# kjedrzejewski/video-cycle_gan-upscaling

Hardware: AMD Instinct MI355X
Metric: upscaled frames/s (train step, G+D fwd+bwd) at 256->512 (higher is better)
Workload: dtype f32; 1 GPU; C2: make_upscaler_orig((512,512,3),k=3,x2,res=9) + PatchGAN-70, batch 8/GPU, gan2 wiring, Wasserstein + pixel-MSE, faithful 3-call step incl. predict pass; global_batch=8, frame=256x256->512x512, parallelism=dp1, launch=hipGraph replay

## Files before the change

video-cycle_gan-upscaling_amd/csrc/conv_transpose.hip:

```cpp
#include "vcg_common.hpp"
#include <type_traits>

namespace {

struct ConvTParams {
    const float* x;
    const float* w;
    float* y;
    const float* bias;
    const float* prelu;
    const float* residual;
    int n, cin, h, w_, cout, oh, ow;
    int tiles_x, tiles_y, co_blocks;
    int act;
    float alpha;
};

constexpr int phase_of(int k, int cb) { return (((k - cb) % 2) + 2) % 2; }
constexpr int d_of(int k, int cb) { return (k - cb - phase_of(k, cb)) / 2; }
constexpr int dmin_of(int K, int cb) { int m = 1000; for (int k = 0; k < K; ++k) m = d_of(k, cb) < m ? d_of(k, cb) : m; return m; }
constexpr int dmax_of(int K, int cb) { int m = -1000; for (int k = 0; k < K; ++k) m = d_of(k, cb) > m ? d_of(k, cb) : m; return m; }

template <int K, int CBY, int CBX, int CK, int MT>
struct ConvTCfg {
    static constexpr int QROWS = 4;
    static constexpr int DMINY = dmin_of(K, CBY), DMAXY = dmax_of(K, CBY);
    static constexpr int DMINX = dmin_of(K, CBX), DMAXX = dmax_of(K, CBX);
    static constexpr int NDY = DMAXY - DMINY + 1, NDX = DMAXX - DMINX + 1;
    static constexpr int NR = QROWS + DMAXY - DMINY;
    static constexpr int NC = 32 + DMAXX - DMINX;
    static constexpr int PLANE = NR * NC;
    static constexpr int T = K * K;
    static constexpr int IN_ELEMS = CK * PLANE;
    static constexpr int MB = 32 * MT;
    static constexpr int W_ELEMS = CK * T * MB;
    static constexpr int IN_PT = (IN_ELEMS + 255) / 256;
    static constexpr int W_PT = (W_ELEMS + 255) / 256;
    static constexpr size_t LDS_BYTES = (size_t)(IN_ELEMS + W_ELEMS) * sizeof(float);
};

template <int K, int CBY, int CBX, int CK, int MT>
__global__ __launch_bounds__(256, (MT == 1 ? 2 : 1)) void convt_kernel(const ConvTParams p) {
    using C = ConvTCfg<K, CBY, CBX, CK, MT>;
    extern __shared__ __attribute__((aligned(16))) float smem[];
    float* s_in = smem;
    float* s_w = smem + C::IN_ELEMS;

    const int tid = threadIdx.x, lane = tid & 63, wv = tid >> 6;
    const int half = lane >> 5, l31 = lane & 31;
    int b = blockIdx.x;
    const int cb = b % p.co_blocks; b /= p.co_blocks;
    const int tx = b % p.tiles_x;   b /= p.tiles_x;
    const int ty = b % p.tiles_y;   b /= p.tiles_y;
    const int n = b;
    const int qx0 = tx * 32, qy0 = ty * C::QROWS, co0 = cb * C::MB;
    const int gy0 = qy0 - C::DMAXY, gx0 = qx0 - C::DMAXX;
    const float* xn = p.x + (size_t)n * p.cin * p.h * p.w_;

    float rin[C::IN_PT], rw[C::W_PT];
    unsigned in_off[C::IN_PT];
#pragma unroll
    for (int i = 0; i < C::IN_PT; ++i) {
        const int e = tid + i * 256;
        unsigned off = VCG_OOB;
        if (e < C::IN_ELEMS) {
            const int ci = e / C::PLANE, rem = e % C::PLANE;
            const int r = rem / C::NC, c = rem % C::NC;
            const int gy = gy0 + r, gx = gx0 + c;
            if (gy >= 0 && gy < p.h && gx >= 0 && gx < p.w_) off = 4u * (unsigned)((ci * p.h + gy) * p.w_ + gx);
        }
        in_off[i] = off;
    }
    const int hw = p.h * p.w_;
    unsigned w_off[C::W_PT];
#pragma unroll
    for (int i = 0; i < C::W_PT; ++i) {
        const int e = tid + i * 256;
        const int m = e % C::MB, q = e / C::MB;
        const int t = q % C::T, ci = q / C::T;
        const int col = co0 + m < p.cout ? co0 + m : p.cout - 1;
        w_off[i] = e < C::W_ELEMS ? 4u * (unsigned)((t * p.cin + ci) * p.cout + col) : VCG_OOB;
    }
    const size_t wbytes = (size_t)C::T * p.cin * p.cout * sizeof(float);
    auto load_chunk = [&](int ci0) {
        const vcg_rsrc rx = make_rsrc(xn + (size_t)ci0 * hw, (size_t)(p.cin - ci0) * hw * sizeof(float));
#pragma unroll
        for (int i = 0; i < C::IN_PT; ++i) rin[i] = buf_load(rx, in_off[i]);
        const vcg_rsrc rwt = make_rsrc(p.w + (size_t)ci0 * p.cout, wbytes - (size_t)ci0 * p.cout * sizeof(float));
#pragma unroll
        for (int i = 0; i < C::W_PT; ++i) rw[i] = buf_load(rwt, w_off[i]);
    };
    auto store_chunk = [&]() {
#pragma unroll
        for (int i = 0; i < C::IN_PT; ++i) {
            const int e = tid + i * 256;
            if (e < C::IN_ELEMS) s_in[e] = rin[i];
        }
#pragma unroll
        for (int i = 0; i < C::W_PT; ++i) {
            const int e = tid + i * 256;
            if (e < C::W_ELEMS) s_w[e] = rw[i];
        }
    };

    f32x16 acc[2][2][MT];
#pragma unroll
    for (int a = 0; a < 2; ++a)
#pragma unroll
        for (int c = 0; c < 2; ++c)
#pragma unroll
            for (int m = 0; m < MT; ++m)
#pragma unroll
                for (int r = 0; r < 16; ++r) acc[a][c][m][r] = 0.f;

    const float* bbase = s_in + half * C::PLANE + wv * C::NC + l31;
    const float* abase = s_w + half * C::T * C::MB + l31;

    const int nchunks = (p.cin + CK - 1) / CK;
    load_chunk(0);
    for (int c = 0; c < nchunks; ++c) {
        __syncthreads();
        store_chunk();
        __syncthreads();
        if (c + 1 < nchunks) load_chunk((c + 1) * CK);
#pragma unroll
        for (int cp = 0; cp < CK / 2; ++cp) {
            float bv[C::NDY][C::NDX];
#pragma unroll
            for (int iy = 0; iy < C::NDY; ++iy)
#pragma unroll
                for (int ix = 0; ix < C::NDX; ++ix)
                    bv[iy][ix] = bbase[cp * 2 * C::PLANE + (C::DMAXY - (C::DMINY + iy)) * C::NC +
                                       (C::DMAXX - (C::DMINX + ix))];
            float av[C::T][MT];
#pragma unroll
            for (int t = 0; t < C::T; ++t)
#pragma unroll
                for (int mt = 0; mt < MT; ++mt) av[t][mt] = abase[(cp * 2 * C::T + t) * C::MB + mt * 32];
#pragma unroll
            for (int ky = 0; ky < K; ++ky) {
#pragma unroll
                for (int kx = 0; kx < K; ++kx) {
                    const int t = ky * K + kx;
                    const int py = phase_of(ky, CBY), px = phase_of(kx, CBX);
                    const int iy = d_of(ky, CBY) - C::DMINY, ix = d_of(kx, CBX) - C::DMINX;
#pragma unroll
                    for (int mt = 0; mt < MT; ++mt) acc[py][px][mt] = mfma32(av[t][mt], bv[iy][ix], acc[py][px][mt]);
                }
            }
        }
    }

    const int qy = qy0 + wv, qx = qx0 + l31;
    const bool vec_ok = (p.ow % 2) == 0;
    const bool full = vec_ok && (co0 + C::MB <= p.cout) && (2 * (qy0 + C::QROWS) <= p.oh) && (2 * (qx0 + 32) <= p.ow);
    const int plane = p.oh * p.ow;
    const size_t img = (size_t)n * p.cout * plane;
    float* yimg = p.y + img;
    const float* rimg = p.residual ? p.residual + img : nullptr;
    const int ob = (co0 + 4 * half) * plane + (2 * qy) * p.ow + 2 * qx;
    const float* bp = p.bias ? p.bias : vcg_zero_word;
    const int bmask = p.bias ? ~0 : 0;
    const bool is_prelu = p.act == VCG_ACT_PRELU;
    const float* ap = is_prelu ? p.prelu : vcg_zero_word;
    const int amask = is_prelu ? ~0 : 0;
    const float slope_u = (p.act == VCG_ACT_LRELU) ? p.alpha : 1.f;
    auto emit = [&](auto guard_tag, auto res_tag) {
        constexpr bool GUARD = decltype(guard_tag)::value, RES = decltype(res_tag)::value;
#pragma unroll
        for (int mt = 0; mt < MT; ++mt) {
#pragma unroll
            for (int r = 0; r < 16; ++r) {
                const int row = mt * 32 + mfma_row(r, lane);
                const int co = co0 + row;
                const bool co_ok = !GUARD || co < p.cout;
                const int cs = co_ok ? co : co0;
                const float bvv = bp[cs & bmask];
                const float pa = ap[cs & amask];
                const float al = is_prelu ? pa : slope_u;
#pragma unroll
                for (int py = 0; py < 2; ++py) {
                    const int o = ob + (row - 4 * half) * plane + py * p.ow;
                    float v0 = acc[py][0][mt][r] + bvv, v1 = acc[py][1][mt][r] + bvv;
                    v0 = v0 >= 0.f ? v0 : v0 * al;
                    v1 = v1 >= 0.f ? v1 : v1 * al;
                    if (!GUARD) {
                        if (RES) { const float2 rr = *reinterpret_cast<const float2*>(rimg + o); v0 += rr.x; v1 += rr.y; }
                        *reinterpret_cast<float2*>(yimg + o) = make_float2(v0, v1);
                    } else {
                        const int oy = 2 * qy + py, ox = 2 * qx;
                        if (co_ok && oy < p.oh && ox < p.ow) {
                            if (vec_ok) {
                                if (RES) { const float2 rr = *reinterpret_cast<const float2*>(rimg + o); v0 += rr.x; v1 += rr.y; }
                                *reinterpret_cast<float2*>(yimg + o) = make_float2(v0, v1);
                            } else {
                                if (RES) v0 += rimg[o];
                                yimg[o] = v0;
                                if (ox + 1 < p.ow) {
                                    if (RES) v1 += rimg[o + 1];
                                    yimg[o + 1] = v1;
                                }
                            }
                        }
                    }
                }
            }
        }
    };
    using T_ = std::true_type;
    using F_ = std::false_type;
    if (full) {
        if (p.residual) emit(F_{}, T_{}); else emit(F_{}, F_{});
    } else {
        if (p.residual) emit(T_{}, T_{}); else emit(T_{}, F_{});
    }
}

template <int K, int CBY, int CBX, int CK, int MT>
int launch_convt(ConvTParams p, hipStream_t st) {
    using C = ConvTCfg<K, CBY, CBX, CK, MT>;
    p.tiles_x = ceil_div(ceil_div(p.ow, 2), 32);
    p.tiles_y = ceil_div(ceil_div(p.oh, 2), C::QROWS);
    p.co_blocks = ceil_div(p.cout, C::MB);
    const long grid = (long)p.tiles_x * p.tiles_y * p.co_blocks * p.n;
    if (grid <= 0 || grid > 0x7fffffffL) return VCG_E_SHAPE;
    auto kern = convt_kernel<K, CBY, CBX, CK, MT>;
    if (int e = vcg_allow_dyn_lds(reinterpret_cast<const void*>(kern), C::LDS_BYTES)) return e;
    hipLaunchKernelGGL(kern, dim3((int)grid), dim3(256), C::LDS_BYTES, st, p);
    VCG_LAUNCH_CHECK();
    return VCG_OK;
}

}

int vcg_internal_convt(const float* x, const float* w, float* y, int n, int cin, int h, int wd, int cout,
                       int oh, int ow, int k, int cby, int cbx, const vcg_epilogue* ep, hipStream_t st) {
    ConvTParams p{};
    p.x = x; p.w = w; p.y = y;
    p.bias = ep ? ep->bias : nullptr;
    p.prelu = ep ? ep->prelu_alpha : nullptr;
    p.residual = ep ? ep->residual : nullptr;
    p.act = ep ? ep->act : VCG_ACT_NONE;
    p.alpha = ep ? ep->act_alpha : 0.f;
    if (p.act == VCG_ACT_PRELU && p.prelu == nullptr) return VCG_E_NULL;
    if (p.act == VCG_ACT_TANH) return VCG_E_UNSUPPORTED;
    p.n = n; p.cin = cin; p.h = h; p.w_ = wd; p.cout = cout; p.oh = oh; p.ow = ow;
    if (n <= 0 || cin <= 0 || cout <= 0 || oh <= 0 || ow <= 0) return VCG_E_SHAPE;
#define VCG_CT(K_, A_, B_, CK_, MT_) if (k == K_ && cby == A_ && cbx == B_) return launch_convt<K_, A_, B_, CK_, MT_>(p, st)
    VCG_CT(3, 0, 0, 16, 1); VCG_CT(3, 0, 1, 16, 1); VCG_CT(3, 1, 0, 16, 1); VCG_CT(3, 1, 1, 16, 1);
    VCG_CT(4, 1, 1, 16, 1);
    VCG_CT(5, 1, 1, 8, 2); VCG_CT(5, 1, 2, 8, 2); VCG_CT(5, 2, 1, 8, 2); VCG_CT(5, 2, 2, 8, 2);
#undef VCG_CT
    return VCG_E_UNSUPPORTED;
}
```

Before: 135.7 frames/s.

## Walk several output-channel blocks per CTA in transposed conv and rework epilogue

Each block now loops over several consecutive output-channel blocks (a walk factor picked from occupancy so the grid still fills the GPU), reusing its input tile position across them. The grid becomes 3D, residual handling becomes a template parameter so the non-residual K=3 kernel can request higher occupancy, and the staging offsets are computed incrementally instead of with divisions. The epilogue uses buffer loads and stores with saturated out-of-bounds offsets, vectorized bias and slope loads, and prefetches the residual. Walking serializes work per block and reloads input chunks per channel block, so it trades parallelism for fewer blocks and less index overhead.

```diff
diff --git a/video-cycle_gan-upscaling_amd/csrc/conv_transpose.hip b/video-cycle_gan-upscaling_amd/csrc/conv_transpose.hip
--- a/video-cycle_gan-upscaling_amd/csrc/conv_transpose.hip
+++ b/video-cycle_gan-upscaling_amd/csrc/conv_transpose.hip
@@ -11,7 +11,8 @@
     const float* prelu;
     const float* residual;
     int n, cin, h, w_, cout, oh, ow;
-    int tiles_x, tiles_y, co_blocks;
+    int tiles_x, co_blocks;
+    int walk;
     int act;
     float alpha;
 };
@@ -39,47 +40,158 @@
     static constexpr size_t LDS_BYTES = (size_t)(IN_ELEMS + W_ELEMS) * sizeof(float);
 };
 
-template <int K, int CBY, int CBX, int CK, int MT>
-__global__ __launch_bounds__(256, (MT == 1 ? 2 : 1)) void convt_kernel(const ConvTParams p) {
+constexpr int CT_OOB = 0x7FFFFFF0;
+__device__ __forceinline__ float2 buf_load2(vcg_rsrc r, int byte_off) {
+    const u32x2 v = __builtin_amdgcn_raw_buffer_load_b64(r, byte_off, 0, 0);
+    return make_float2(__uint_as_float(v.x), __uint_as_float(v.y));
+}
+__device__ __forceinline__ f32x4 buf_load4(vcg_rsrc r, int byte_off) {
+    return __builtin_bit_cast(f32x4, __builtin_amdgcn_raw_buffer_load_b128(r, byte_off, 0, 0));
+}
+__device__ __forceinline__ void buf_store2(vcg_rsrc r, int byte_off, float a, float b) {
+    u32x2 v;
+    v.x = __float_as_uint(a);
+    v.y = __float_as_uint(b);
+    __builtin_amdgcn_raw_buffer_store_b64(v, r, byte_off, 0, 0);
+}
+
+template <int MT, bool RES>
+__device__ __forceinline__ void convt_epilogue(const ConvTParams& p, f32x16 (&acc)[2][2][MT], int n, int co0, int qy, int qx, int half) {
+    constexpr int MB = 32 * MT;
+    const int plane = p.oh * p.ow, plane4 = 4 * plane, ow4 = 4 * p.ow;
+    const int nch = p.cout - co0 < MB ? p.cout - co0 : MB;
+    const size_t blk = ((size_t)n * p.cout + co0) * plane;
+    const size_t blk_bytes = (size_t)nch * plane * sizeof(float);
+    const vcg_rsrc ry = make_rsrc(p.y + blk, blk_bytes);
+    const vcg_rsrc rr = make_rsrc(RES ? p.residual + blk : nullptr, RES ? blk_bytes : 0);
+    const bool is_prelu = p.act == VCG_ACT_PRELU;
+    const vcg_rsrc rbias = make_rsrc(p.bias, p.bias ? (size_t)p.cout * sizeof(float) : 0);
+    const vcg_rsrc rslope = make_rsrc(is_prelu ? p.prelu : nullptr, is_prelu ? (size_t)p.cout * sizeof(float) : 0);
+    const float slope_u = (p.act == VCG_ACT_LRELU) ? p.alpha : 1.f;
+    const int chan4 = 4 * (co0 + 4 * half);
+
+    const int base = (4 * half) * plane4 + (2 * qy) * ow4 + 8 * qx;
+    int vo[2][2];
+#pragma unroll
+    for (int py = 0; py < 2; ++py)
+#pragma unroll
+        for (int px = 0; px < 2; ++px)
+            vo[py][px] = (2 * qy + py < p.oh && 2 * qx + px < p.ow) ? base + py * ow4 + 4 * px : CT_OOB;
+    asm volatile("" : "+v"(vo[0][0]), "+v"(vo[0][1]), "+v"(vo[1][0]), "+v"(vo[1][1]));
+
+    constexpr int NG = 4 * MT;
+    auto emit = [&](auto vec_tag) {
+        constexpr bool VEC = decltype(vec_tag)::value;
+        float rs[2][4][2][2];
+        auto row_of = [](int g, int j) { return (g >> 2) * 32 + 8 * (g & 3) + j; };
+        auto load_res = [&](int g) {
+#pragma unroll
+            for (int j = 0; j < 4; ++j) {
+                const int srow = row_of(g, j) * plane4;
+#pragma unroll
+                for (int py = 0; py < 2; ++py) {
+                    if (VEC) {
+                        const float2 v = buf_load2(rr, __builtin_elementwise_add_sat(vo[py][0], srow));
+                        rs[g & 1][j][py][0] = v.x;
+                        rs[g & 1][j][py][1] = v.y;
+                    } else {
+                        rs[g & 1][j][py][0] = buf_load(rr, (unsigned)__builtin_elementwise_add_sat(vo[py][0], srow));
+                        rs[g & 1][j][py][1] = buf_load(rr, (unsigned)__builtin_elementwise_add_sat(vo[py][1], srow));
+                    }
+                }
+            }
+        };
+        if (RES) load_res(0);
+#pragma unroll
+        for (int g = 0; g < NG; ++g) {
+            const f32x4 bv = buf_load4(rbias, chan4 + 4 * row_of(g, 0));
+            const f32x4 pa = buf_load4(rslope, chan4 + 4 * row_of(g, 0));
+            if (RES && g + 1 < NG) load_res(g + 1);
+#pragma unroll
+            for (int j = 0; j < 4; ++j) {
+                const int mt = g >> 2, r = 4 * (g & 3) + j;
+                const int srow = row_of(g, j) * plane4;
+                const float al = is_prelu ? pa[j] : slope_u;
+#pragma unroll
+                for (int py = 0; py < 2; ++py) {
+                    float v0 = acc[py][0][mt][r] + bv[j], v1 = acc[py][1][mt][r] + bv[j];
+                    v0 = v0 >= 0.f ? v0 : v0 * al;
+                    v1 = v1 >= 0.f ? v1 : v1 * al;
+                    if (RES) { v0 += rs[g & 1][j][py][0]; v1 += rs[g & 1][j][py][1]; }
+                    if (VEC) {
+                        buf_store2(ry, __builtin_elementwise_add_sat(vo[py][0], srow), v0, v1);
+                    } else {
+                        buf_store(ry, (unsigned)__builtin_elementwise_add_sat(vo[py][0], srow), v0);
+                        buf_store(ry, (unsigned)__builtin_elementwise_add_sat(vo[py][1], srow), v1);
+                    }
+                }
+            }
+            __builtin_amdgcn_sched_barrier(0);
+        }
+    };
+    if ((p.ow & 1) == 0) emit(std::true_type{}); else emit(std::false_type{});
+}
+
+template <int K, int CBY, int CBX, int CK, int MT, bool RES>
+__global__ __launch_bounds__(256, (MT == 1 ? (K == 3 && !RES ? 3 : 2) : 1)) void convt_kernel(const ConvTParams p) {
     using C = ConvTCfg<K, CBY, CBX, CK, MT>;
+    static_assert(C::W_ELEMS % 256 == 0 && 256 % C::MB == 0, "every thread stages W_PT weights of one column");
     extern __shared__ __attribute__((aligned(16))) float smem[];
     float* s_in = smem;
     float* s_w = smem + C::IN_ELEMS;
 
     const int tid = threadIdx.x, lane = tid & 63, wv = tid >> 6;
     const int half = lane >> 5, l31 = lane & 31;
-    int b = blockIdx.x;
-    const int cb = b % p.co_blocks; b /= p.co_blocks;
-    const int tx = b % p.tiles_x;   b /= p.tiles_x;
-    const int ty = b % p.tiles_y;   b /= p.tiles_y;
-    const int n = b;
-    const int qx0 = tx * 32, qy0 = ty * C::QROWS, co0 = cb * C::MB;
+    const int groups = p.co_blocks / p.walk;
+    const int tx = blockIdx.x / groups, cb0 = (blockIdx.x - tx * groups) * p.walk;
+    const int ty = blockIdx.y, n = blockIdx.z;
+    const int qx0 = tx * 32, qy0 = ty * C::QROWS;
     const int gy0 = qy0 - C::DMAXY, gx0 = qx0 - C::DMAXX;
     const float* xn = p.x + (size_t)n * p.cin * p.h * p.w_;
+    const int hw = p.h * p.w_;
 
     float rin[C::IN_PT], rw[C::W_PT];
     unsigned in_off[C::IN_PT];
-#pragma unroll
-    for (int i = 0; i < C::IN_PT; ++i) {
-        const int e = tid + i * 256;
-        unsigned off = VCG_OOB;
-        if (e < C::IN_ELEMS) {
-            const int ci = e / C::PLANE, rem = e % C::PLANE;
-            const int r = rem / C::NC, c = rem % C::NC;
-            const int gy = gy0 + r, gx = gx0 + c;
-            if (gy >= 0 && gy < p.h && gx >= 0 && gx < p.w_) off = 4u * (unsigned)((ci * p.h + gy) * p.w_ + gx);
-        }
-        in_off[i] = off;
+    {
+        constexpr int Q1 = 256 / C::PLANE, R1 = 256 % C::PLANE, QR = R1 / C::NC, RC = R1 % C::NC;
+        const unsigned w4 = 4u * (unsigned)p.w_, hw4 = 4u * (unsigned)hw;
+        const unsigned step = (unsigned)Q1 * hw4 + (unsigned)QR * w4 + 4u * RC;
+        const unsigned col_wrap = w4 - 4u * C::NC, row_wrap = hw4 - (unsigned)C::NR * w4;
+        int ci = tid / C::PLANE, r = (tid % C::PLANE) / C::NC, c = (tid % C::PLANE) % C::NC;
+        unsigned off = (unsigned)ci * hw4 + (unsigned)(gy0 + r) * w4 + 4u * (unsigned)(gx0 + c);
+#pragma unroll
+        for (int i = 0; i < C::IN_PT; ++i) {
+            const bool in_tile = (i + 1) * 256 <= C::IN_ELEMS || ci < CK;
+            const bool ok = in_tile && (unsigned)(gy0 + r) < (unsigned)p.h && (unsigned)(gx0 + c) < (unsigned)p.w_;
+            in_off[i] = ok ? off : VCG_OOB;
+            c += RC;
+            const bool cw = c >= C::NC;
+            c -= cw ? C::NC : 0;
+            r += QR + (cw ? 1 : 0);
+            const bool rwr = r >= C::NR;
+            r -= rwr ? C::NR : 0;
+            ci += Q1 + (rwr ? 1 : 0);
+            off += step + (cw ? col_wrap : 0u) + (rwr ? row_wrap : 0u);
+        }
     }
-    const int hw = p.h * p.w_;
     unsigned w_off[C::W_PT];
-#pragma unroll
-    for (int i = 0; i < C::W_PT; ++i) {
-        const int e = tid + i * 256;
-        const int m = e % C::MB, q = e / C::MB;
-        const int t = q % C::T, ci = q / C::T;
-        const int col = co0 + m < p.cout ? co0 + m : p.cout - 1;
-        w_off[i] = e < C::W_ELEMS ? 4u * (unsigned)((t * p.cin + ci) * p.cout + col) : VCG_OOB;
+    const int wm = tid % C::MB;
+    auto w_col = [&](int co0) { return 4u * (unsigned)(co0 + wm < p.cout ? co0 + wm : p.cout - 1); };
+    {
+        constexpr int QS = 256 / C::MB, QC = QS / C::T, QT = QS % C::T;
+        const unsigned cout4 = 4u * (unsigned)p.cout, tap4 = (unsigned)p.cin * cout4;
+        const unsigned step = (unsigned)QT * tap4 + (unsigned)QC * cout4, wrap = cout4 - (unsigned)C::T * tap4;
+        int t = (tid / C::MB) % C::T, ci = (tid / C::MB) / C::T;
+        unsigned off = (unsigned)t * tap4 + (unsigned)ci * cout4 + w_col(cb0 * C::MB);
+#pragma unroll
+        for (int i = 0; i < C::W_PT; ++i) {
+            w_off[i] = off;
+            t += QT;
+            const bool tw = t >= C::T;
+            t -= tw ? C::T : 0;
+            ci += QC + (tw ? 1 : 0);
+            off += step + (tw ? wrap : 0u);
+        }
     }
     const size_t wbytes = (size_t)C::T * p.cin * p.cout * sizeof(float);
     auto load_chunk = [&](int ci0) {
@@ -97,136 +209,103 @@
             if (e < C::IN_ELEMS) s_in[e] = rin[i];
         }
 #pragma unroll
-        for (int i = 0; i < C::W_PT; ++i) {
-            const int e = tid + i * 256;
-            if (e < C::W_ELEMS) s_w[e] = rw[i];
-        }
+        for (int i = 0; i < C::W_PT; ++i) s_w[tid + i * 256] = rw[i];
     };
-
-    f32x16 acc[2][2][MT];
-#pragma unroll
-    for (int a = 0; a < 2; ++a)
-#pragma unroll
-        for (int c = 0; c < 2; ++c)
-#pragma unroll
-            for (int m = 0; m < MT; ++m)
-#pragma unroll
-                for (int r = 0; r < 16; ++r) acc[a][c][m][r] = 0.f;
 
     const float* bbase = s_in + half * C::PLANE + wv * C::NC + l31;
     const float* abase = s_w + half * C::T * C::MB + l31;
 
     const int nchunks = (p.cin + CK - 1) / CK;
     load_chunk(0);
-    for (int c = 0; c < nchunks; ++c) {
-        __syncthreads();
-        store_chunk();
-        __syncthreads();
-        if (c + 1 < nchunks) load_chunk((c + 1) * CK);
-#pragma unroll
-        for (int cp = 0; cp < CK / 2; ++cp) {
-            float bv[C::NDY][C::NDX];
-#pragma unroll
-            for (int iy = 0; iy < C::NDY; ++iy)
-#pragma unroll
-                for (int ix = 0; ix < C::NDX; ++ix)
-                    bv[iy][ix] = bbase[cp * 2 * C::PLANE + (C::DMAXY - (C::DMINY + iy)) * C::NC +
-                                       (C::DMAXX - (C::DMINX + ix))];
-            float av[C::T][MT];
-#pragma unroll
-            for (int t = 0; t < C::T; ++t)
-#pragma unroll
-                for (int mt = 0; mt < MT; ++mt) av[t][mt] = abase[(cp * 2 * C::T + t) * C::MB + mt * 32];
-#pragma unroll
-            for (int ky = 0; ky < K; ++ky) {
-#pragma unroll
-                for (int kx = 0; kx < K; ++kx) {
-                    const int t = ky * K + kx;
-                    const int py = phase_of(ky, CBY), px = phase_of(kx, CBX);
-                    const int iy = d_of(ky, CBY) - C::DMINY, ix = d_of(kx, CBX) - C::DMINX;
-#pragma unroll
-                    for (int mt = 0; mt < MT; ++mt) acc[py][px][mt] = mfma32(av[t][mt], bv[iy][ix], acc[py][px][mt]);
-                }
-            }
-        }
-    }
-
-    const int qy = qy0 + wv, qx = qx0 + l31;
-    const bool vec_ok = (p.ow % 2) == 0;
-    const bool full = vec_ok && (co0 + C::MB <= p.cout) && (2 * (qy0 + C::QROWS) <= p.oh) && (2 * (qx0 + 32) <= p.ow);
-    const int plane = p.oh * p.ow;
-    const size_t img = (size_t)n * p.cout * plane;
-    float* yimg = p.y + img;
-    const float* rimg = p.residual ? p.residual + img : nullptr;
-    const int ob = (co0 + 4 * half) * plane + (2 * qy) * p.ow + 2 * qx;
-    const float* bp = p.bias ? p.bias : vcg_zero_word;
-    const int bmask = p.bias ? ~0 : 0;
-    const bool is_prelu = p.act == VCG_ACT_PRELU;
-    const float* ap = is_prelu ? p.prelu : vcg_zero_word;
-    const int amask = is_prelu ? ~0 : 0;
-    const float slope_u = (p.act == VCG_ACT_LRELU) ? p.alpha : 1.f;
-    auto emit = [&](auto guard_tag, auto res_tag) {
-        constexpr bool GUARD = decltype(guard_tag)::value, RES = decltype(res_tag)::value;
-#pragma unroll
-        for (int mt = 0; mt < MT; ++mt) {
-#pragma unroll
-            for (int r = 0; r < 16; ++r) {
-                const int row = mt * 32 + mfma_row(r, lane);
-                const int co = co0 + row;
-                const bool co_ok = !GUARD || co < p.cout;
-                const int cs = co_ok ? co : co0;
-                const float bvv = bp[cs & bmask];
-                const float pa = ap[cs & amask];
-                const float al = is_prelu ? pa : slope_u;
-#pragma unroll
-                for (int py = 0; py < 2; ++py) {
-                    const int o = ob + (row - 4 * half) * plane + py * p.ow;
-                    float v0 = acc[py][0][mt][r] + bvv, v1 = acc[py][1][mt][r] + bvv;
-                    v0 = v0 >= 0.f ? v0 : v0 * al;
-                    v1 = v1 >= 0.f ? v1 : v1 * al;
-                    if (!GUARD) {
-                        if (RES) { const float2 rr = *reinterpret_cast<const float2*>(rimg + o); v0 += rr.x; v1 += rr.y; }
-                        *reinterpret_cast<float2*>(yimg + o) = make_float2(v0, v1);
-                    } else {
-                        const int oy = 2 * qy + py, ox = 2 * qx;
-                        if (co_ok && oy < p.oh && ox < p.ow) {
-                            if (vec_ok) {
-                                if (RES) { const float2 rr = *reinterpret_cast<const float2*>(rimg + o); v0 += rr.x; v1 += rr.y; }
-                                *reinterpret_cast<float2*>(yimg + o) = make_float2(v0, v1);
-                            } else {
-                                if (RES) v0 += rimg[o];
-                                yimg[o] = v0;
-                                if (ox + 1 < p.ow) {
-                                    if (RES) v1 += rimg[o + 1];
-                                    yimg[o + 1] = v1;
-                                }
-                            }
-                        }
+    for (int wb = 0; wb < p.walk; ++wb) {
+        const int co0 = (cb0 + wb) * C::MB;
+        f32x16 acc[2][2][MT];
+#pragma unroll
+        for (int a = 0; a < 2; ++a)
+#pragma unroll
+            for (int c = 0; c < 2; ++c)
+#pragma unroll
+                for (int m = 0; m < MT; ++m)
+#pragma unroll
+                    for (int r = 0; r < 16; ++r) acc[a][c][m][r] = 0.f;
+
+        for (int c = 0; c < nchunks; ++c) {
+            __syncthreads();
+            store_chunk();
+            __syncthreads();
+            if (c + 1 < nchunks) load_chunk((c + 1) * CK);
+#pragma unroll
+            for (int cp = 0; cp < CK / 2; ++cp) {
+                float bv[C::NDY][C::NDX];
+#pragma unroll
+                for (int iy = 0; iy < C::NDY; ++iy)
+#pragma unroll
+                    for (int ix = 0; ix < C::NDX; ++ix)
+                        bv[iy][ix] = bbase[cp * 2 * C::PLANE + (C::DMAXY - (C::DMINY + iy)) * C::NC +
+                                           (C::DMAXX - (C::DMINX + ix))];
+                float av[C::T][MT];
+#pragma unroll
+                for (int t = 0; t < C::T; ++t)
+#pragma unroll
+                    for (int mt = 0; mt < MT; ++mt) av[t][mt] = abase[(cp * 2 * C::T + t) * C::MB + mt * 32];
+#pragma unroll
+                for (int ky = 0; ky < K; ++ky) {
+#pragma unroll
+                    for (int kx = 0; kx < K; ++kx) {
+                        const int t = ky * K + kx;
+                        const int py = phase_of(ky, CBY), px = phase_of(kx, CBX);
+                        const int iy = d_of(ky, CBY) - C::DMINY, ix = d_of(kx, CBX) - C::DMINX;
+#pragma unroll
+                        for (int mt = 0; mt < MT; ++mt) acc[py][px][mt] = mfma32(av[t][mt], bv[iy][ix], acc[py][px][mt]);
                     }
                 }
             }
         }
-    };
-    using T_ = std::true_type;
-    using F_ = std::false_type;
-    if (full) {
-        if (p.residual) emit(F_{}, T_{}); else emit(F_{}, F_{});
-    } else {
-        if (p.residual) emit(T_{}, T_{}); else emit(T_{}, F_{});
+        convt_epilogue<MT, RES>(p, acc, n, co0, qy0 + wv, qx0 + l31, half);
+        if (wb + 1 < p.walk) {
+            const unsigned dcol = w_col(co0 + C::MB) - w_col(co0);
+#pragma unroll
+            for (int i = 0; i < C::W_PT; ++i) w_off[i] += dcol;
+            load_chunk(0);
+        }
     }
 }
 
-template <int K, int CBY, int CBX, int CK, int MT>
+bool convt_block_fits(int mb, int oh, int ow, int ck, int h, int w, int taps, int cin, int cout) {
+    return (unsigned long long)mb * oh * ow * sizeof(float) < 0x7FFFFFE0ull && (unsigned long long)ck * h * w * sizeof(float) < 0xFFFFFFE0ull &&
+           (unsigned long long)taps * cin * cout * sizeof(float) < 0xFFFFFFE0ull;
+}
+
+template <typename Kern>
+int resident_slots(Kern kern, size_t lds) {
+    int dev = 0, cus = 0, per_cu = 0;
+    if (hipGetDevice(&dev) != hipSuccess || hipDeviceGetAttribute(&cus, hipDeviceAttributeMultiprocessorCount, dev) != hipSuccess) return 0;
+    if (hipOccupancyMaxActiveBlocksPerMultiprocessor(&per_cu, kern, 256, lds) != hipSuccess) return 0;
+    return cus > 0 && per_cu > 0 ? cus * per_cu : 0;
+}
+
+int pick_walk(int co_blocks, long tiles, int slots) {
+    if (slots <= 0) return 1;
+    for (int d = co_blocks; d > 1; --d)
+        if (co_blocks % d == 0 && tiles * (co_blocks / d) >= 4L * slots) return d;
+    return 1;
+}
+
+template <int K, int CBY, int CBX, int CK, int MT, bool RES>
 int launch_convt(ConvTParams p, hipStream_t st) {
     using C = ConvTCfg<K, CBY, CBX, CK, MT>;
+    if (!convt_block_fits(C::MB, p.oh, p.ow, CK, p.h, p.w_, C::T, p.cin, p.cout)) return VCG_E_UNSUPPORTED;
     p.tiles_x = ceil_div(ceil_div(p.ow, 2), 32);
-    p.tiles_y = ceil_div(ceil_div(p.oh, 2), C::QROWS);
+    const int tiles_y = ceil_div(ceil_div(p.oh, 2), C::QROWS);
     p.co_blocks = ceil_div(p.cout, C::MB);
-    const long grid = (long)p.tiles_x * p.tiles_y * p.co_blocks * p.n;
-    if (grid <= 0 || grid > 0x7fffffffL) return VCG_E_SHAPE;
-    auto kern = convt_kernel<K, CBY, CBX, CK, MT>;
+    if (tiles_y > 65535 || p.n > 65535) return VCG_E_SHAPE;
+    auto kern = convt_kernel<K, CBY, CBX, CK, MT, RES>;
     if (int e = vcg_allow_dyn_lds(reinterpret_cast<const void*>(kern), C::LDS_BYTES)) return e;
-    hipLaunchKernelGGL(kern, dim3((int)grid), dim3(256), C::LDS_BYTES, st, p);
+    static const int slots = resident_slots(kern, C::LDS_BYTES);
+    p.walk = pick_walk(p.co_blocks, (long)p.tiles_x * tiles_y * p.n, slots);
+    const long gx = (long)p.tiles_x * (p.co_blocks / p.walk);
+    if (gx <= 0 || gx > 0x7fffffffL) return VCG_E_SHAPE;
+    hipLaunchKernelGGL(kern, dim3((int)gx, tiles_y, p.n), dim3(256), C::LDS_BYTES, st, p);
     VCG_LAUNCH_CHECK();
     return VCG_OK;
 }
@@ -246,7 +325,7 @@
     if (p.act == VCG_ACT_TANH) return VCG_E_UNSUPPORTED;
     p.n = n; p.cin = cin; p.h = h; p.w_ = wd; p.cout = cout; p.oh = oh; p.ow = ow;
     if (n <= 0 || cin <= 0 || cout <= 0 || oh <= 0 || ow <= 0) return VCG_E_SHAPE;
-#define VCG_CT(K_, A_, B_, CK_, MT_) if (k == K_ && cby == A_ && cbx == B_) return launch_convt<K_, A_, B_, CK_, MT_>(p, st)
+#define VCG_CT(K_, A_, B_, CK_, MT_) if (k == K_ && cby == A_ && cbx == B_) return p.residual ? launch_convt<K_, A_, B_, CK_, MT_, true>(p, st) : launch_convt<K_, A_, B_, CK_, MT_, false>(p, st)
     VCG_CT(3, 0, 0, 16, 1); VCG_CT(3, 0, 1, 16, 1); VCG_CT(3, 1, 0, 16, 1); VCG_CT(3, 1, 1, 16, 1);
     VCG_CT(4, 1, 1, 16, 1);
     VCG_CT(5, 1, 1, 8, 2); VCG_CT(5, 1, 2, 8, 2); VCG_CT(5, 2, 1, 8, 2); VCG_CT(5, 2, 2, 8, 2);
```

New measurement: 136.3 frames/s (median of 6 runs). Within noise of the previous version (+0.4%).
